# ethz-asl/infinitam

Hardware: AMD Instinct MI355X
Metric: fused depth frames/sec (640x480, hash TSDF) (higher is better)
Workload: dtype f32

## Files before the change

### include/itm_debug.h

```cpp
#ifndef ITM_DEBUG_H_
#define ITM_DEBUG_H_

#include "itm_hip.h"

#ifdef __cplusplus
extern "C" {
#endif

#define ITM_DEBUG_FORCE_GLOBAL_RANGE_ATOMICS 1
#define ITM_DEBUG_EXPLICIT_MARK_PREVIOUS 2
#define ITM_DEBUG_INTEGRATE_WORKGROUPS 3
#define ITM_DEBUG_NO_FUSED_PROJECTION 4
#define ITM_DEBUG_NO_DIRECTORY 5
#define ITM_DEBUG_NO_FUSED_RANGE_REDUCE 6
#define ITM_DEBUG_TWO_PASS_VISIBLE_LIST 7
#define ITM_DEBUG_SINGLE_PASS_RAYCAST 8
#define ITM_DEBUG_DENSE_GROUP_CULL 9
#define ITM_DEBUG_TRACKER_LAUNCH_PER_EVALUATION 10
#define ITM_DEBUG_TRACKER_HOST_COMMAND 11
#define ITM_DEBUG_SEPARATE_SWEEP 13
#define ITM_DEBUG_NO_SIDE_PROJECTION 14
#define ITM_DEBUG_DENSE_RANGE_REFILL 15
#define ITM_DEBUG_NO_SDF_MIRROR 12
#define ITM_DEBUG_DENSE_CLASSIFY 16
#define ITM_DEBUG_DENSE_NO_STRIPS 17
#define ITM_DEBUG_TRACKER_SESSION_UNUSABLE 18
#define ITM_DEBUG_NO_DEFERRED_FUSION 19
#define ITM_DEBUG_FORCE_LIST_STUCK 20
#define ITM_DEBUG_EXCHANGE_DEVICE_COPY 24
#define ITM_DEBUG_EXCHANGE_CORRUPT_WORD 25
#define ITM_DEBUG_MESH_ATTR_PER_VERTEX 26
#define ITM_DEBUG_MESH_INDEX_WEAK_HASH 27
int ITM_FN(debug_set)(int key, int value);
int ITM_FN(debug_checksum)(const int32_t* src, size_t words, int rounds, unsigned long long* dst, itm_stream stream);
int ITM_FN(debug_dense_classify_check)(int32_t out[4], int reset);
int ITM_FN(debug_column_cull_rows)(const float M_d[16], const float intr[4], int w, int h, float voxelSize, const int size[3],
                                   const int offset[3], int x0, int z, int* rlo, int* rhi);
int ITM_FN(debug_div32767)(const float* in, float* out, int n, itm_stream stream);
int ITM_FN(debug_divide)(int mode, const float* a, const float* b, const float* r, float* out, int n, itm_stream stream);


typedef int (*itm_icp_evaluate_fn)(void* user, int level, int iterationType, const float approxInvPose[16],
                                   float distThresh, itm_tracker_gh* out);
int ITM_FN(debug_icp_track)(const itm_tracker_config* cfg, const float M_d[16], itm_icp_evaluate_fn evaluate,
                            void* user, float M_d_out[16]);
int ITM_FN(debug_wicp_track)(const itm_tracker_config* cfg, const float M_d[16], itm_icp_evaluate_fn evaluate,
                             void* user, float M_d_out[16]);

#ifdef __cplusplus
}
#endif
#endif
```

### infinitam_amd/capi.py

```python
from __future__ import annotations

import ctypes as C
import os
import re
from dataclasses import dataclass, field
from typing import Optional

import numpy as np

VOXEL_S, VOXEL_F, VOXEL_S_RGB, VOXEL_F_RGB = 0, 1, 2, 3
INDEX_HASH, INDEX_DENSE = 0, 1
RENDER_SHADED_GREYSCALE, RENDER_COLOUR_FROM_VOLUME, RENDER_COLOUR_FROM_NORMAL = 0, 1, 2
(BUF_HASH_ENTRIES, BUF_EXCESS_LIST, BUF_VOXEL_BLOCKS, BUF_ALLOCATION_LIST, BUF_VISIBLE_IDS,
 BUF_VISIBLE_TYPE, BUF_RANGE_IMAGE, BUF_RAYCAST_RESULT, BUF_RAYCAST_IMAGE, BUF_FORWARD_PROJECTION,
 BUF_MISSING_POINTS, BUF_SWAP_STATES) = range(12)
ERR_INVALID, ERR_DEVICE, ERR_UNSUPPORTED = -1, -2, -3
MESH_NORMALS, MESH_COLOURS = 1, 2

VOXEL_NAMES = {VOXEL_S: "ITMVoxel_s", VOXEL_F: "ITMVoxel_f", VOXEL_S_RGB: "ITMVoxel_s_rgb",
               VOXEL_F_RGB: "ITMVoxel_f_rgb"}

HASH_ENTRY_DTYPE = np.dtype({"names": ["pos", "offset", "ptr"],
                             "formats": [("<i2", 3), "<i4", "<i4"],
                             "offsets": [0, 8, 12], "itemsize": 16})
# ... 211 lines not shown
    "host_free": (C.c_int, [_P]),
    "host_register": (C.c_int, [_P, C.c_size_t]),
    "host_unregister": (C.c_int, [_P]),
    "depth_stager_create": (C.c_int, [C.c_int, C.c_int, C.c_int, C.POINTER(_P)]),
    "depth_stager_destroy": (C.c_int, [_P]),
    "depth_stager_upload": (C.c_int, [_P, _P]),
    "depth_stager_acquire": (C.c_int, [_P, _P, C.POINTER(_P)]),
    "depth_stager_release": (C.c_int, [_P, _P]),
    "depth_stager_set_conversion": (C.c_int, [_P, C.c_int, C.c_float, C.c_float, C.c_float]),
    "depth_stager_acquire_depth": (C.c_int, [_P, _P, C.POINTER(_P), C.POINTER(_P)]),
    "depth_stager_pending": (C.c_int, [_P, C.POINTER(C.c_int), C.POINTER(C.c_int)]),
    "stream_create": (C.c_int, [C.POINTER(_P)]),
    "stream_destroy": (C.c_int, [_P]),
    "exchange_unique_id": (C.c_int, [C.POINTER(C.c_ubyte)]),
    "exchange_create": (C.c_int, [C.c_int, C.c_int, C.POINTER(C.c_ubyte), C.c_int, C.c_int, C.POINTER(_P)]),
    "exchange_destroy": (C.c_int, [_P]),
    "exchange_step": (C.c_int, [_P, _P, C.POINTER(C.c_float), _P]),
    "exchange_info": (C.c_int, [_P, C.POINTER(C.c_int), C.POINTER(C.c_int), C.POINTER(C.c_int), C.POINTER(C.c_int), C.POINTER(_P)]),
    "exchange_table": (C.c_int, [_P, _P, C.c_size_t]),
    "exchange_self_check": (C.c_int, [_P, C.POINTER(C.c_int), C.POINTER(C.c_int)]),
    "exchange_acquire": (C.c_int, [_P, _P, C.POINTER(_P), C.POINTER(C.c_longlong)]),
    "exchange_release": (C.c_int, [_P, _P]),
    "debug_checksum": (C.c_int, [_P, C.c_size_t, C.c_int, _P, _P]),
    "colour_tracker_create": (C.c_int, [C.POINTER(_P)]),
    "colour_tracker_destroy": (C.c_int, [_P]),
    "colour_tracker_prepare": (C.c_int, [_P, C.POINTER(ViewStruct), C.c_int, _P]),
    "colour_tracker_read_level": (C.c_int, [_P, C.c_int, _P, _P, _P, C.POINTER(C.c_int), C.POINTER(C.c_int), _P]),
    "colour_tracker_evaluate": (C.c_int, [_P, C.c_int, _P, _P, C.c_int, C.POINTER(C.c_float), C.c_int, C.c_int, C.POINTER(ColourEval), _P]),
    "colour_tracker_track_camera": (C.c_int, [_P, C.POINTER(TrackerConfig), C.POINTER(ViewStruct), _P, _P, _P, C.c_int,
                                              C.POINTER(C.c_float), _P]),
    "colour_tracker_evaluations": (C.c_int, [_P, C.POINTER(C.c_int)]),
    "ren_tracker_create": (C.c_int, [C.POINTER(_P)]),
    "ren_tracker_destroy": (C.c_int, [_P]),
    "ren_tracker_prepare": (C.c_int, [_P, C.POINTER(ViewStruct), _P, _P]),
    "ren_tracker_evaluate": (C.c_int, [_P, _P, C.POINTER(C.c_float), C.c_int, C.POINTER(RenEval), _P]),
    "ren_tracker_track_camera": (C.c_int, [_P, _P, C.POINTER(ViewStruct), C.POINTER(C.c_float), C.POINTER(C.c_int), _P]),
    "mesh_attributes": (C.c_int, [_P, _P, C.c_int, _P]),
    "mesh_download_attributes": (C.c_int, [_P, _P, _P, C.c_uint32, C.POINTER(C.c_uint32), _P]),
    "mesh_write_ply": (C.c_int, [_P, C.c_char_p, _P]),
    "mesh_index": (C.c_int, [_P, _P]),
    "mesh_index_info": (C.c_int, [_P, C.POINTER(C.c_uint32), C.POINTER(C.c_uint32), C.POINTER(_P), C.POINTER(_P), C.POINTER(_P), _P]),
    "mesh_download_indexed": (C.c_int, [_P, _P, _P, C.c_uint32, _P, C.c_uint32, C.POINTER(C.c_uint32), C.POINTER(C.c_uint32), _P]),
    "mesh_indexed_attributes": (C.c_int, [_P, _P, C.c_int, _P]),
    "mesh_download_indexed_attributes": (C.c_int, [_P, _P, _P, C.c_uint32, C.POINTER(C.c_uint32), _P]),
    "mesh_write_ply_indexed": (C.c_int, [_P, C.c_char_p, _P]),
    "mesh_write_obj_indexed": (C.c_int, [_P, C.c_char_p, _P]),
# ... 482 lines not shown
```

### infinitam_amd/csrc/itm_internal.h

```cpp
#pragma once

#include <hip/hip_runtime.h>

#include <string>
#include <vector>

#include "../../include/itm_hip.h"
#include "../../include/itm_debug.h"
#include "itm_types.h"

namespace itm {

struct SceneCounters {
  int32_t lastFreeBlockId;
  int32_t lastFreeExcessListId;
  int32_t noAllocRequests;
  int32_t statusFlags;
};
struct RenderCounters {
  int32_t noVisibleEntries;
  int32_t noFwdProjMissingPoints;
  int32_t noTotalPoints;
  int32_t noRenderingBlocks;
  int32_t rawVisibleCount;
// ... 65 lines not shown

struct itm_render_state {
  const itm_scene* scene = nullptr;
  int w = 0, h = 0;
  bool hash = false;
  int capIds = 0;
  bool listCoherent = true;
  bool lazyThisFrame = false;
  float2* range = nullptr;
  float4* raycast = nullptr;
  float4* fwdProj = nullptr;
  int32_t* missing = nullptr;
  uchar4* image = nullptr;
  int32_t* visibleIds = nullptr;
  uint8_t* visibleType = nullptr;
  itm::RenderCounters* counters = nullptr;
  uint4* projBuf = nullptr;
  uint2* rangePartials = nullptr;
  int32_t* pixScratch = nullptr;
  int32_t* pixChunk = nullptr;
  uint8_t* viewFlags = nullptr;
  int32_t* viewChunkVis = nullptr;
  bool denseRangeReady = false;
  hipStream_t sideStream = nullptr;
  hipEvent_t listReady = nullptr, projectionDone = nullptr;
  struct { bool valid = false; const float* depth = nullptr; int w = 0, h = 0; float M_d[16] = {}, intr_d[4] = {}; bool lazy = false; unsigned tableEpoch = 0; } ahead;
  struct { int stage = 0; itm_view view = {}; hipStream_t st = nullptr; } deferred;
};

namespace itm {

int set_error(int code, const std::string& msg);
int hip_fail(hipError_t e, const char* what, const char* file, int line);

#define ITM_HIP(call)                                                        \
  do {                                                                       \
    hipError_t _e = (call);                                                  \
    if (_e != hipSuccess) return itm::hip_fail(_e, #call, __FILE__, __LINE__); \
  } while (0)

#define ITM_LAUNCH_CHECK()                                                    \
  do {                                                                        \
    hipError_t _e = hipGetLastError();                                        \
    if (_e != hipSuccess) return itm::hip_fail(_e, "kernel launch", __FILE__, __LINE__); \
  } while (0)

// ... 26 lines not shown
int flush_deferred(itm_render_state* rs);
int enter_scene(const itm_scene* s, const itm_render_state* rs);
int flush_overlapping(const void* p, size_t bytes, hipStream_t st);
void forget_deferred(itm_render_state* rs);
extern int g_debug_no_deferred_fusion;
bool deferred_fusion_default();
extern int g_debug_force_list_stuck;
extern int g_debug_exchange_device_copy, g_debug_exchange_corrupt_word;
extern int g_debug_mesh_attr_per_vertex;
extern int g_debug_mesh_index_weak_hash;
int refuse_while_ahead(const itm_scene* s, const itm_render_state* rs, const char* what);

extern int g_debug_explicit_mark;
extern int g_debug_two_pass_visible_list;
extern int g_debug_integrate_wgs;
extern int g_debug_dense_group_cull;
extern int g_debug_dense_classify;
extern int g_debug_dense_no_strips;
extern int g_debug_tracker_launch_per_evaluation;
extern int g_debug_tracker_host_command;
extern int g_debug_tracker_session_unusable;
extern int g_debug_no_sdf_mirror;
extern int g_debug_separate_sweep;
int rebuild_sdf_mirror(itm_scene* s, hipStream_t st);
int launch_swap_after_allocation(itm_scene* s, itm_render_state* rs, hipStream_t st);
void free_swap_state(itm_scene* s);
int create_swap_state(itm_scene* s);
int live_hash_scenes(int device);
int accel_unfill(itm_scene* s, hipStream_t st);
int accel_place(itm_scene* s, const float* invM, hipStream_t st);
extern int g_debug_no_fused_projection;
int rebuild_head_bits(itm_scene* s, hipStream_t st);
extern int g_debug_no_directory;
int launch_request_stage(itm_scene* s, const itm_view* v, itm_render_state* rs, bool onlyVisible, bool fuseRangeInit, hipStream_t st);
int launch_sweep_stage(itm_scene* s, const itm_view* v, itm_render_state* rs, bool onlyVisible, hipStream_t st);
int launch_allocate(itm_scene* s, const itm_view* v, itm_render_state* rs, bool onlyVisible, bool fuseRangeInit, hipStream_t st);
int validate_allocate(const itm_scene* s, const itm_view* v, const itm_render_state* rs, bool onlyVisible);
int validate_integrate(const itm_scene* s, const itm_view* v);
int cancel_ahead(itm_scene* s, itm_render_state* rs, hipStream_t st);
int launch_integrate(itm_scene* s, const itm_view* v, itm_render_state* rs, hipStream_t st, bool fuseProjection = false);
bool can_fuse_projection(const itm_scene* s, const itm_render_state* rs);
int launch_find_visible(const itm_scene* s, const float* M, const float* intr, itm_render_state* rs, hipStream_t st);
int launch_expected_depths(const itm_scene* s, const float* M, const float* intr, itm_render_state* rs, bool rangeAlreadyInit, hipStream_t st, bool projected = false);
int launch_raycast(const itm_scene* s, const float* invM, const float* intr, itm_render_state* rs, float4* dst, hipStream_t st, bool reduceRange = false);
int launch_icp_maps(const itm_scene* s, const itm_view* v, itm_render_state* rs, float4* points, float4* normals, hipStream_t st, bool reduceRange = false,
                    itm_scene* sceneForNext = nullptr, const itm_view* next = nullptr);
// ... 6 lines not shown
```

### infinitam_amd/csrc/scene.hip

```cpp
#include <atomic>
#include <mutex>
#include <cstdio>
#include <cstring>
#include <new>

#include "itm_internal.h"

namespace itm {

static thread_local std::string g_last_error;

int set_error(int code, const std::string& msg) {
  g_last_error = msg;
  return code;
}
int hip_fail(hipError_t e, const char* what, const char* file, int line) {
  char buf[512];
  snprintf(buf, sizeof buf, "%s: %s (%s:%d)", what, hipGetErrorString(e), file, line);
  g_last_error = buf;
  return ITM_ERR_DEVICE;
}

hipEvent_t Profiler::get() {
  if (!pool.empty()) { hipEvent_t e = pool.back(); pool.pop_back(); return e; }
// ... 342 lines not shown
  (void)hipFree(s->hash); (void)hipFree(s->excessList); (void)hipFree(s->vba); (void)hipFree(s->allocList);
  (void)hipFree(s->counters); (void)hipFree(s->headBits); (void)hipFree(s->allocKey); (void)hipFree(s->chunkReq); (void)hipFree(s->chunkVis); (void)hipFree(s->chunkGran); (void)hipFree(s->chunkSweepDone); (void)hipFree(s->chunkKeptGran);
  (void)hipFree(s->dirPtr); (void)hipFree(s->dirSlot); (void)hipFree(s->sdfMirror); (void)hipFree(s->org.mTable); (void)hipFree(s->org.mPages); (void)hipFree(s->depthTiles);
  delete s;
}
static void free_rs(itm_render_state* r) {
  if (!r) return;
  bool haveScene;
  { std::lock_guard<std::mutex> lock(g_rsRegistryMutex); haveScene = r->scene != nullptr; }
  if (haveScene) (void)flush_deferred(r);
  {
    std::lock_guard<std::mutex> lock(g_rsRegistryMutex);
    itm_scene* s = const_cast<itm_scene*>(r->scene);
    if (s) {
      if (s->aheadRs == r) s->aheadRs = nullptr;
      for (size_t i = 0; i < s->renderStates.size(); ++i)
        if (s->renderStates[i] == r) { s->renderStates[i] = s->renderStates.back(); s->renderStates.pop_back(); break; }
    }
  }
  forget_deferred(r);
  (void)hipFree(r->range); (void)hipFree(r->raycast); (void)hipFree(r->fwdProj); (void)hipFree(r->missing);
  (void)hipFree(r->image); (void)hipFree(r->visibleIds); (void)hipFree(r->visibleType); (void)hipFree(r->counters);
  (void)hipFree(r->projBuf); (void)hipFree(r->rangePartials); (void)hipFree(r->pixScratch); (void)hipFree(r->pixChunk); (void)hipFree(r->viewFlags); (void)hipFree(r->viewChunkVis);
  if (r->sideStream) { (void)hipStreamSynchronize(r->sideStream); (void)hipStreamDestroy(r->sideStream); }
  if (r->listReady) (void)hipEventDestroy(r->listReady);
  if (r->projectionDone) (void)hipEventDestroy(r->projectionDone);
  delete r;
}

}

using namespace itm;

extern "C" {

const char* itm_version(void) { return "itm-hip 0.1 (gfx950)"; }
const char* itm_last_error(void) { return g_last_error.c_str(); }
int itm_uses_device_memory(void) { return 1; }
size_t itm_voxel_size_bytes(int t) {
  switch (t) {
    case ITM_VOXEL_S: return VoxelS::kBytes;
    case ITM_VOXEL_F: return VoxelF::kBytes;
    case ITM_VOXEL_S_RGB: return VoxelSRgb::kBytes;
    case ITM_VOXEL_F_RGB: return VoxelFRgb::kBytes;
  }
  return 0;
// ... 202 lines not shown

int itm_reset_scene(itm_scene* s, itm_stream stream) {
  if (!s) return set_error(ITM_ERR_INVALID, "null scene");
  hipStream_t st = as_stream(stream);
  if (s->deferredRs) { const int rc = flush_deferred(s->deferredRs); if (rc) return rc; }
  if (s->aheadRs) { const int rc = cancel_ahead(s, s->aheadRs, st); if (rc) return rc; }
  if (s->fatalHost && *s->fatalHost) { ITM_HIP(hipStreamSynchronize(st)); *s->fatalHost = 0; }
  const int grid = 2048;
  if (s->cfg.voxelType == ITM_VOXEL_S && (s->numVoxels % 4) == 0) {
    reset_voxels_s_x4_kernel<<<grid, 256, 0, st>>>((uint4*)s->vba, s->numVoxels / 4);
  } else {
    int rc = dispatch_voxel(s->cfg.voxelType, [&](auto vx) {
      using VX = decltype(vx);
      reset_voxels_kernel<VX><<<grid, 256, 0, st>>>(s->vba, s->numVoxels);
      return ITM_OK;
    });
    if (rc) return rc;
  }
  ITM_LAUNCH_CHECK();
  if (s->cfg.indexType == ITM_INDEX_HASH) {
    { int rc = accel_unfill(s, st); if (rc) return rc; }
    s->orgPlaced = false;
    ++s->tableEpoch;
    reset_hash_kernel<<<1024, 256, 0, st>>>(s->hash, s->noTotalEntries, s->excessList, s->cfg.excessNum, s->allocList,
                                            s->cfg.localBlockNum, s->allocKey, s->headBits, (s->cfg.bucketNum + 31) / 32, s->chunkReq, s->numChunks * 4, s->counters);
  } else {
    reset_dense_kernel<<<1, 1, 0, st>>>(s->allocList, s->counters);
  }
  ITM_LAUNCH_CHECK();
  return ITM_OK;
}

int itm_render_state_create(const itm_scene* s, int w, int h, itm_render_state** out) {
  if (!s || !out || w <= 0 || h <= 0) return set_error(ITM_ERR_INVALID, "bad argument");
  if ((long long)w * h >= (1ll << 24)) return set_error(ITM_ERR_INVALID, "image too large");
  itm_render_state* r = new (std::nothrow) itm_render_state();
  if (!r) return set_error(ITM_ERR_DEVICE, "out of host memory");
  r->scene = s; r->w = w; r->h = h;
  r->hash = s->cfg.indexType == ITM_INDEX_HASH;
  r->capIds = r->hash ? s->cfg.localBlockNum : 0;
  size_t P = (size_t)w * h;
  hipError_t e = hipSuccess;
  auto alloc = [&](void** p, size_t bytes) { if (e == hipSuccess) e = hipMalloc(p, bytes ? bytes : 16); };
  alloc((void**)&r->range, P * 8);
  alloc((void**)&r->raycast, P * 16);
  alloc((void**)&r->fwdProj, P * 16);
  alloc((void**)&r->missing, P * 4);
  alloc((void**)&r->image, P * 4);
  alloc((void**)&r->counters, sizeof(RenderCounters));
  alloc((void**)&r->pixScratch, P * 4);
  alloc((void**)&r->pixChunk, ((P + kSweepChunk - 1) / kSweepChunk) * 4 + 16);
  if (r->hash) {
    alloc((void**)&r->visibleIds, (size_t)r->capIds * 4);
    alloc((void**)&r->visibleType, (size_t)s->noTotalEntries);
    alloc((void**)&r->projBuf, (size_t)r->capIds * 32);
    if ((size_t)((w + 7) / 8) * ((h + 7) / 8) * 8 <= 150 * 1024) alloc((void**)&r->rangePartials, (size_t)64 * ((w + 7) / 8) * ((h + 7) / 8) * 8);
  }
  if (e != hipSuccess) { free_rs(r); return hip_fail(e, "hipMalloc(render state)", __FILE__, __LINE__); }
  e = hipMemset(r->counters, 0, sizeof(RenderCounters));
  if (e == hipSuccess) e = hipMemset(r->raycast, 0, P * 16);
  if (e == hipSuccess) e = hipMemset(r->fwdProj, 0, P * 16);
  if (e == hipSuccess) e = hipMemset(r->missing, 0, P * 4);
  if (e == hipSuccess) e = hipMemset(r->image, 0, P * 4);
  if (e == hipSuccess && r->hash) e = hipMemset(r->visibleIds, 0, (size_t)r->capIds * 4);
  if (e == hipSuccess && r->hash) e = hipMemset(r->visibleType, 0, (size_t)s->noTotalEntries);
  if (e != hipSuccess) { free_rs(r); return hip_fail(e, "hipMemset(render state)", __FILE__, __LINE__); }
  fill_range_kernel<<<256, 256, 0, 0>>>(r->range, (int)P, s->prm.viewFrustum_min, s->prm.viewFrustum_max);
  e = hipDeviceSynchronize();
  if (e != hipSuccess) { free_rs(r); return hip_fail(e, "init range image", __FILE__, __LINE__); }
  { std::lock_guard<std::mutex> lock(g_rsRegistryMutex); s->renderStates.push_back(r); }
  *out = r;
  return ITM_OK;
}
int itm_render_state_destroy(itm_render_state* r) { free_rs(r); return ITM_OK; }

int itm_debug_div32767(const float* in, float* out, int n, itm_stream st) {
  if (!in || !out || n < 0) return set_error(ITM_ERR_INVALID, "bad argument");
  div32767_kernel<<<(n + 255) / 256, 256, 0, as_stream(st)>>>(in, out, n);
  ITM_LAUNCH_CHECK();
  return ITM_OK;
}

int itm_debug_divide(int mode, const float* a, const float* b, const float* r, float* out, int n, itm_stream st) {
  if (!a || !b || !out || n < 0 || mode < 1 || mode > 4 || (mode == 4 && !r)) return set_error(ITM_ERR_INVALID, "bad argument");
  divide_kernel<<<(n + 255) / 256, 256, 0, as_stream(st)>>>(mode, a, b, r, out, n);
  ITM_LAUNCH_CHECK();
  return ITM_OK;
}
// ... 154 lines not shown
```

### infinitam_amd/csrc/visualise.hip

```cpp
#include <cstdlib>
#include <cstring>

#include "itm_internal.h"
#include "alloc_device.h"
#include "shading_device.h"
#include "range_device.h"
#include "wave_utils.h"


namespace itm {

#ifndef ITM_MIRROR_FLOAT_TYPES
#define ITM_MIRROR_FLOAT_TYPES 0
#endif

int g_debug_force_global_range = 0;
int g_debug_no_directory = 0;
int g_debug_no_sdf_mirror = 0;
int g_debug_no_fused_range_reduce = 0;
int g_debug_single_pass_raycast = 0;
int g_debug_no_side_projection = 0;
int g_debug_dense_range_refill = 0;

__global__ void __launch_bounds__(256) range_init_kernel(float2* __restrict__ img, int n, float a, float b, RenderCounters* rc) {
  const int stride = gridDim.x * blockDim.x;
  for (int i = blockIdx.x * blockDim.x + threadIdx.x; i < n; i += stride) img[i] = make_float2(a, b);
  if (blockIdx.x == 0 && threadIdx.x == 0) { rc->noRenderingBlocks = 0; rc->renderingBlocksAccepted = -1; }
}

__device__ inline void merge_box(float2* __restrict__ range, int W, const Projected& r) {
  const uint32_t z0 = __float_as_uint(r.z0), z1 = __float_as_uint(r.z1);
  for (int y = r.uly; y <= r.lry; ++y)
    for (int x = r.ulx; x <= r.lrx; ++x) {
      uint32_t* px = (uint32_t*)&range[x + y * W];
      atomicMin(px, z0);
      atomicMax(px + 1, z1);
    }
}

__global__ void __launch_bounds__(256) project_fill_kernel(const int32_t* __restrict__ ids, RenderCounters* __restrict__ rc,
                                                           const uint4* __restrict__ hash, float2* __restrict__ range,
                                                           uint4* __restrict__ projBuf, ProjParams p) {
  const int nv = rc->noVisibleEntries;
// ... 206 lines not shown
  __syncthreads();
  if (tid < 4) {
    const int cx = tx * 2 + (tid & 1), cy = ty * 2 + (tid >> 1);
    const float2 r = make_float2(__uint_as_float(capCells[2 * tid]), __uint_as_float(capCells[2 * tid + 1]));
    cellRange[tid] = r;
    if (cx < f.RW && cy < f.RH) f.range[cx + cy * W] = r;
  }
}

constexpr float kSilhouetteSpread = 0.3f;
constexpr int kSilhouettePrio = 3;
#ifndef ITM_EXP_RAYCAST_STAMPS
#define ITM_EXP_RAYCAST_STAMPS 0
#endif
#if ITM_EXP_RAYCAST_STAMPS
__device__ unsigned long long g_rayStamps[8192 * 4];
#define ITM_RS(...) __VA_ARGS__
#else
#define ITM_RS(...)
#endif

struct AheadRequest { RequestArgs ra; AllocParams ap; int rayTiles, reqTilesX; };

template <class VX, bool DENSE, bool REDUCE, bool PARK, bool AHEAD = false, int MIRROR = 0>
__global__ void __launch_bounds__(256) raycast_kernel(VolumeView volIn, const float2* __restrict__ range, float4* __restrict__ out, RayParams p, RangeFuse fuse, AheadRequest ahead) {
  if constexpr (AHEAD) {
    if ((int)blockIdx.x >= ahead.rayTiles) {
      const int r = (int)blockIdx.x - ahead.rayTiles;
      request_tile<false, false, true>(r % ahead.reqTilesX, r / ahead.reqTilesX, ahead.ra, ahead.ap);
      return;
    }
  }
  VolumeViewM<MIRROR> vol(volIn);
  if constexpr (MIRROR == 0) vol.sdfMirror = nullptr;
  const int lane = threadIdx.x & 63, wave = threadIdx.x >> 6;
  const int tilesX = (p.W + 15) / 16;
  const int tx = blockIdx.x % tilesX, ty = blockIdx.x / tilesX;
  const int lx = lane & 15, ly = wave * 4 + (lane >> 4);
  const int x = tx * 16 + lx;
  const int y = ty * 16 + ly;
  const bool inside = x < p.W && y < p.H;
  __shared__ float2 cellRange[4];
  __shared__ float4 parkState[PARK ? 256 : 1];
  __shared__ int parkSource[PARK ? 256 : 1];
  __shared__ int parkCount;
  if (PARK && threadIdx.x == 0) parkCount = 0;
  ITM_RS(unsigned long long* stamp = g_rayStamps + (size_t)((blockIdx.x * 4 + wave) & 8191) * 4; if (lane == 0) stamp[0] = __builtin_amdgcn_s_memrealtime();)
  float2 mm = make_float2(0.0f, 0.0f);
  if constexpr (REDUCE) {
    reduce_own_cells(fuse, tx, ty, p.W, cellRange);
    __syncthreads();
    if (inside) mm = cellRange[(lx >> 3) + 2 * (ly >> 3)];
  } else {
    if (PARK) __syncthreads();
    if (inside) mm = range[(x >> 3) + (y >> 3) * p.W];
  }
  ITM_RS(if (lane == 0) stamp[1] = __builtin_amdgcn_s_memrealtime();)
  if (!DENSE && __any(inside && mm.y - mm.x > kSilhouetteSpread)) __builtin_amdgcn_s_setprio(kSilhouettePrio);
  bool parked = false;
  if (inside) {
// ... 1 lines not shown
    if (!parked) out[x + y * p.W] = r;
    else if constexpr (PARK) {
      const int slot = atomicAdd(&parkCount, 1);
      parkState[slot] = r;
      parkSource[slot] = ly * 16 + lx;
    }
  }
  ITM_RS(if (lane == 0) { stamp[2] = __builtin_amdgcn_s_memrealtime(); stamp[3] = 0; })
  if constexpr (PARK) {
    __syncthreads();
    const int n = parkCount;
    if ((int)threadIdx.x < n) {
      const float4 q = parkState[threadIdx.x];
      const int src = parkSource[threadIdx.x];
      const int qx = tx * 16 + (src & 15), qy = ty * 16 + (src >> 4);
      float2 m2;
      if constexpr (REDUCE) m2 = cellRange[((src & 15) >> 3) + 2 * (src >> 7)];
      else m2 = range[(qx >> 3) + (qy >> 3) * p.W];
      const RayResume rr{q.x, q.y, q.z, q.w};
      bool again;
      out[qx + qy * p.W] = march_ray<VX, DENSE, kParkedLookahead, false>(qx, qy, vol, p, m2, &rr, again);
    }
    ITM_RS(if (lane == 0) stamp[3] = __builtin_amdgcn_s_memrealtime() | ((unsigned long long)(wave == 0 ? n : 0) << 52);)
  }
}
#if ITM_EXP_RAYCAST_STAMPS
extern "C" int itm_debug_read_raycast_stamps(unsigned long long* dst, int n) { return (int)hipMemcpyFromSymbol(dst, HIP_SYMBOL(g_rayStamps), (size_t)n * 8); }
#endif

int launch_raycast(const itm_scene* s, const float* invM, const float* intr, itm_render_state* rs, float4* dst, hipStream_t st, bool reduceRange, const AheadRequest* aheadIn) {
  RayParams p; make_ray_params(s, invM, intr, rs->w, rs->h, p);
  const VolumeView vol = make_volume(s);
  const int rayTiles = ((rs->w + 15) / 16) * ((rs->h + 15) / 16);
  const bool dense = s->cfg.indexType == ITM_INDEX_DENSE;
  RangeFuse fuse{rs->rangePartials, rs->counters, rs->projBuf, rs->range, (rs->w + 7) / 8, (rs->h + 7) / 8, s->cfg.maxRenderingBlocks};
  const bool park = !dense && vol.dirPtr != nullptr && !g_debug_single_pass_raycast;
  AheadRequest ahead;
  memset(&ahead, 0, sizeof ahead);
  int reqTiles = 0;
  if (aheadIn && !dense) { ahead = *aheadIn; ahead.rayTiles = rayTiles; reqTiles = ahead.reqTilesX * ((ahead.ap.H + 15) / 16); }
  const dim3 grid(rayTiles + reqTiles);
  KernelTimer tk(s, ITM_TK_RAYCAST, st);
  const int mirrorForm = (!vol.sdfMirror || !park) ? 0 : (vol.org.mMaxPages < 0 ? 1 : 2);
  int rc = dispatch_voxel(s->cfg.voxelType, [&](auto vx) {
    using VX = decltype(vx);
    constexpr bool kMayMirror = VX::kShort || ITM_MIRROR_FLOAT_TYPES;
#define ITM_RC(RED, PRK, AHD, MIR) raycast_kernel<VX, false, RED, PRK, AHD, MIR><<<grid, 256, 0, st>>>(vol, rs->range, dst, p, fuse, ahead)
#define ITM_RC_MIRROR(RED, AHD) do { if (kMayMirror && mirrorForm == 1) ITM_RC(RED, true, AHD, (kMayMirror ? 1 : 0)); else if (kMayMirror && mirrorForm == 2) ITM_RC(RED, true, AHD, (kMayMirror ? 2 : 0)); else ITM_RC(RED, true, AHD, 0); } while (0)
    if (dense) raycast_kernel<VX, true, false, false><<<grid, 256, 0, st>>>(vol, rs->range, dst, p, fuse, ahead);
    else if (reqTiles) {
      if (park) { if (reduceRange) ITM_RC_MIRROR(true, true); else ITM_RC_MIRROR(false, true); }
      else if (reduceRange) ITM_RC(true, false, true, 0);
      else ITM_RC(false, false, true, 0);
    }
    else if (park) { if (reduceRange) ITM_RC_MIRROR(true, false); else ITM_RC_MIRROR(false, false); }
    else if (reduceRange) ITM_RC(true, false, false, 0);
    else ITM_RC(false, false, false, 0);
#undef ITM_RC_MIRROR
#undef ITM_RC
    return ITM_OK;
  });
  if (rc) return rc;
  ITM_LAUNCH_CHECK();
  return ITM_OK;
}
int launch_raycast(const itm_scene* s, const float* invM, const float* intr, itm_render_state* rs, float4* dst, hipStream_t st, bool reduceRange) {
  return launch_raycast(s, invM, intr, rs, dst, st, reduceRange, nullptr);
}

__device__ inline void nt_store(float4* p, float4 v) { __builtin_nontemporal_store(v.x, &p->x); __builtin_nontemporal_store(v.y, &p->y); __builtin_nontemporal_store(v.z, &p->z); __builtin_nontemporal_store(v.w, &p->w); }
__device__ inline void nt_store(uchar4* p, uchar4 v) { __builtin_nontemporal_store(*(unsigned int*)&v, (unsigned int*)p); }

__global__ void __launch_bounds__(256) icp_maps_kernel(const float4* __restrict__ rays, float4* __restrict__ points,
                                                       float4* __restrict__ normals, uchar4* __restrict__ image, RayParams p) {
  __shared__ float4 hits[20][20];
  const int lane = threadIdx.x & 63, wave = threadIdx.x >> 6;
  const int lx = lane & 15, ly = wave * 4 + (lane >> 4);
  const int x = blockIdx.x * 16 + lx, y = blockIdx.y * 16 + ly;
  const bool inside = x < p.W && y < p.H;
  if (inside) hits[2 + ly][2 + lx] = rays[x + y * p.W];
  if (threadIdx.x < 128) {
    const int strip = threadIdx.x >> 5, k = threadIdx.x & 31;
    int hx, hy;
    if (strip < 2) { hx = strip == 0 ? (k & 1) : 18 + (k & 1); hy = 2 + (k >> 1); }
    else { hy = strip == 2 ? (k & 1) : 18 + (k & 1); hx = 2 + (k >> 1); }
    const int gx = (int)blockIdx.x * 16 + hx - 2, gy = (int)blockIdx.y * 16 + hy - 2;
    if (gx >= 0 && gx < p.W && gy >= 0 && gy < p.H) hits[hy][hx] = rays[gx + gy * p.W];
  }
  __syncthreads();
  if (!inside) return;
  const int loc = x + y * p.W;
  const float4 r = hits[2 + ly][2 + lx];
  bool found = r.w > 0.0f;
  float nx = 0, ny = 0, nz = 0, angle = 0;
  const int ox = (int)blockIdx.x * 16 - 2, oy = (int)blockIdx.y * 16 - 2;
  if (found) found = normal_from_hits_at([&](int qx, int qy) { return hits[qy - oy][qx - ox]; }, x, y, p.W, p.H, p.voxelSize, p.lx, p.ly, p.lz, nx, ny, nz, angle);
  if (found) {
    nt_store(&image[loc], grey_pixel(angle));
    nt_store(&points[loc], make_float4(r.x * p.voxelSize, r.y * p.voxelSize, r.z * p.voxelSize, 1.0f));
    nt_store(&normals[loc], make_float4(nx, ny, nz, 0.0f));
  } else {
    const float4 inv = make_float4(0.0f, 0.0f, 0.0f, -1.0f);
    nt_store(&points[loc], inv); nt_store(&normals[loc], inv); nt_store(&image[loc], make_uchar4(0, 0, 0, 0));
  }
}

__global__ void __launch_bounds__(256) icp_maps_init_next_kernel(const float4* __restrict__ rays, float4* __restrict__ points, float4* __restrict__ normals,
                                                                 uchar4* __restrict__ image, RayParams p, float2* __restrict__ range, RenderCounters* __restrict__ rcnt) {
  const int lane = threadIdx.x & 63, wave = threadIdx.x >> 6;
  if (blockIdx.x == 0 && blockIdx.y == 0 && threadIdx.x == 0) { rcnt->noRenderingBlocks = 0; rcnt->renderingBlocksAccepted = -1; }
  const int x = blockIdx.x * 16 + (lane & 15);
  const int y = blockIdx.y * 16 + wave * 4 + (lane >> 4);
  if (x >= p.W || y >= p.H) return;
  const int loc = x + y * p.W;
  range[loc] = make_float2(999999.9f, 0.05f);
  const float4 r = rays[loc];
  bool found = r.w > 0.0f;
  float nx = 0, ny = 0, nz = 0, angle = 0;
  if (found) found = normal_from_hits(rays, x, y, p.W, p.H, p.voxelSize, p.lx, p.ly, p.lz, nx, ny, nz, angle);
  if (found) {
    nt_store(&image[loc], grey_pixel(angle));
    nt_store(&points[loc], make_float4(r.x * p.voxelSize, r.y * p.voxelSize, r.z * p.voxelSize, 1.0f));
    nt_store(&normals[loc], make_float4(nx, ny, nz, 0.0f));
  } else {
    const float4 inv = make_float4(0.0f, 0.0f, 0.0f, -1.0f);
    nt_store(&points[loc], inv); nt_store(&normals[loc], inv); nt_store(&image[loc], make_uchar4(0, 0, 0, 0));
  }
}

int prepare_request_stage(itm_scene* s, const itm_view* v, itm_render_state* rs, hipStream_t st, AllocParams& p, RequestArgs& ra, bool& lazy);

int launch_icp_maps(const itm_scene* s, const itm_view* v, itm_render_state* rs, float4* points, float4* normals, hipStream_t st, bool reduceRange,
                    itm_scene* sceneForNext, const itm_view* next) {
  float invM[16];
  if (!invert4(v->M_d, invM)) return set_error(ITM_ERR_INVALID, "pose matrix is singular");
  AheadRequest ahead;
  bool issueAhead = false;
  if (next && sceneForNext) {
    bool lazy = false;
    int rc = prepare_request_stage(sceneForNext, next, rs, st, ahead.ap, ahead.ra, lazy);
    if (rc) return rc;
    issueAhead = lazy;
    ahead.reqTilesX = (next->w + 15) / 16;
  }
  int rc = launch_raycast(s, invM, v->intr_d, rs, rs->raycast, st, reduceRange, issueAhead ? &ahead : nullptr);
  if (rc) return rc;
  RayParams p; make_ray_params(s, invM, v->intr_d, rs->w, rs->h, p);
  const dim3 grid((rs->w + 15) / 16, (rs->h + 15) / 16);
  KernelTimer tk(s, ITM_TK_ICP_MAPS, st);
  if (issueAhead) {
    icp_maps_init_next_kernel<<<grid, 256, 0, st>>>(rs->raycast, points, normals, rs->image, p, rs->range, rs->counters);
    rs->ahead.tableEpoch = sceneForNext->tableEpoch;
    sceneForNext->aheadRs = rs;
    rs->ahead.valid = true; rs->ahead.depth = next->depth; rs->ahead.w = next->w; rs->ahead.h = next->h; rs->ahead.lazy = true;
    memcpy(rs->ahead.M_d, next->M_d, 64); memcpy(rs->ahead.intr_d, next->intr_d, 16);
  } else {
    icp_maps_kernel<<<grid, 256, 0, st>>>(rs->raycast, points, normals, rs->image, p);
  }
  ITM_LAUNCH_CHECK();
  return ITM_OK;
}

template <class VX, bool DENSE>
__global__ void __launch_bounds__(256) render_image_kernel(VolumeView vol, const float4* __restrict__ rays, uchar4* __restrict__ out, int type, RayParams p) {
  const int lane = threadIdx.x & 63, wave = threadIdx.x >> 6;
  const int x = blockIdx.x * 16 + (lane & 15);
  const int y = blockIdx.y * 16 + wave * 4 + (lane >> 4);
  if (x >= p.W || y >= p.H) return;
  const int loc = x + y * p.W;
  const float4 r = rays[loc];
  bool found = r.w > 0;
  float nx = 0, ny = 0, nz = 0, angle = 0;
  if (found) found = normal_from_sdf<VX, DENSE>(vol, r.x, r.y, r.z, p, nx, ny, nz, angle);
  if (!found) { out[loc] = make_uchar4(0, 0, 0, 0); return; }
  if (type == ITM_RENDER_COLOUR_FROM_VOLUME) {
    const float4 c = colour_at<VX, DENSE>(vol, r.x, r.y, r.z);
    out[loc] = make_uchar4((unsigned char)(c.x * 255.0f), (unsigned char)(c.y * 255.0f), (unsigned char)(c.z * 255.0f), 255);
  } else if (type == ITM_RENDER_COLOUR_FROM_NORMAL) {
    unsigned char* o = (unsigned char*)&out[loc];
    o[0] = (unsigned char)((0.3f + (-nx + 1.0f) * 0.35f) * 255.0f);
    o[1] = (unsigned char)((0.3f + (-ny + 1.0f) * 0.35f) * 255.0f);
    o[2] = (unsigned char)((0.3f + (-nz + 1.0f) * 0.35f) * 255.0f);
// ... 36 lines not shown
  if (key == ITM_DEBUG_EXPLICIT_MARK_PREVIOUS) { g_debug_explicit_mark = value; return ITM_OK; }
  if (key == ITM_DEBUG_INTEGRATE_WORKGROUPS) { g_debug_integrate_wgs = value; return ITM_OK; }
  if (key == ITM_DEBUG_NO_FUSED_PROJECTION) { g_debug_no_fused_projection = value; return ITM_OK; }
  if (key == ITM_DEBUG_NO_DIRECTORY) { g_debug_no_directory = value; return ITM_OK; }
  if (key == ITM_DEBUG_NO_FUSED_RANGE_REDUCE) { g_debug_no_fused_range_reduce = value; return ITM_OK; }
  if (key == ITM_DEBUG_TWO_PASS_VISIBLE_LIST) { g_debug_two_pass_visible_list = value; return ITM_OK; }
  if (key == ITM_DEBUG_SINGLE_PASS_RAYCAST) { g_debug_single_pass_raycast = value; return ITM_OK; }
  if (key == ITM_DEBUG_DENSE_GROUP_CULL) { g_debug_dense_group_cull = value; return ITM_OK; }
  if (key == ITM_DEBUG_TRACKER_LAUNCH_PER_EVALUATION) { g_debug_tracker_launch_per_evaluation = value; return ITM_OK; }
  if (key == ITM_DEBUG_TRACKER_HOST_COMMAND) { g_debug_tracker_host_command = value; return ITM_OK; }
  if (key == ITM_DEBUG_NO_SDF_MIRROR) { g_debug_no_sdf_mirror = value; return ITM_OK; }
  if (key == ITM_DEBUG_SEPARATE_SWEEP) { g_debug_separate_sweep = value; return ITM_OK; }
  if (key == ITM_DEBUG_NO_SIDE_PROJECTION) { g_debug_no_side_projection = value; return ITM_OK; }
  if (key == ITM_DEBUG_DENSE_RANGE_REFILL) { g_debug_dense_range_refill = value; return ITM_OK; }
  if (key == ITM_DEBUG_DENSE_CLASSIFY) { g_debug_dense_classify = value; return ITM_OK; }
  if (key == ITM_DEBUG_TRACKER_SESSION_UNUSABLE) { g_debug_tracker_session_unusable = value; return ITM_OK; }
  if (key == ITM_DEBUG_DENSE_NO_STRIPS) { g_debug_dense_no_strips = value; return ITM_OK; }
  if (key == ITM_DEBUG_NO_DEFERRED_FUSION) { g_debug_no_deferred_fusion = value; return ITM_OK; }
  if (key == ITM_DEBUG_FORCE_LIST_STUCK) { g_debug_force_list_stuck = value; return ITM_OK; }
  if (key == ITM_DEBUG_EXCHANGE_DEVICE_COPY) { g_debug_exchange_device_copy = value; return ITM_OK; }
  if (key == ITM_DEBUG_EXCHANGE_CORRUPT_WORD) { g_debug_exchange_corrupt_word = value; return ITM_OK; }
  if (key == ITM_DEBUG_MESH_ATTR_PER_VERTEX) { g_debug_mesh_attr_per_vertex = value; return ITM_OK; }
  if (key == ITM_DEBUG_MESH_INDEX_WEAK_HASH) { g_debug_mesh_index_weak_hash = value; return ITM_OK; }
  return set_error(ITM_ERR_INVALID, "unknown debug key");
}

int itm_find_surface(const itm_scene* s, const float M[16], const float intr[4], itm_render_state* rs, itm_stream stream) {
  if (!s || !M || !intr || !rs) return set_error(ITM_ERR_INVALID, "null argument");
  if (rs->scene != s) return set_error(ITM_ERR_INVALID, "render state belongs to another scene");
  { const int rc = enter_scene(s, rs); if (rc) return rc; }
  float invM[16];
  if (!invert4(M, invM)) return set_error(ITM_ERR_INVALID, "pose matrix is singular");
  return launch_raycast(s, invM, intr, rs, rs->raycast, as_stream(stream));
}

int itm_render_image(const itm_scene* s, const float M[16], const float intr[4], itm_render_state* rs, uint8_t* out, int type, itm_stream stream) {
  if (!s || !M || !intr || !rs) return set_error(ITM_ERR_INVALID, "null argument");
  if (rs->scene != s) return set_error(ITM_ERR_INVALID, "render state belongs to another scene");
  { const int rc = enter_scene(s, rs); if (rc) return rc; }
  return launch_render_image(s, M, intr, rs, out ? (uchar4*)out : rs->image, type, as_stream(stream));
}

int itm_process_frame(itm_scene* s, const itm_view* v, itm_render_state* rs, float* points, float* normals, itm_stream stream) {
  return itm_process_frame_ahead(s, v, nullptr, rs, points, normals, stream);
}

int itm_process_frame_ahead(itm_scene* s, const itm_view* v, const itm_view* next, itm_render_state* rs, float* points, float* normals, itm_stream stream) {
// ... 31 lines not shown
```

Baseline: 12680.

## Reorder raycast tiles so previously slow tiles dispatch first

The parked raycast kernel records per tile whether any rays needed the slow parked path. The last block of the ICP-maps kernel then builds a permutation that puts those flagged tiles first, and the next frame's raycast reads its tile index from that permutation. The aim is to start long-running tiles early and shorten the tail of unbalanced workgroups. The cost is an extra indirection per block, a serial per-thread scan in one block, and a dependence on frame-to-frame coherence. The order is invalidated when the hash table is reset.

```diff
diff --git a/include/itm_debug.h b/include/itm_debug.h
--- a/include/itm_debug.h
+++ b/include/itm_debug.h
@@ -31,7 +31,9 @@
 #define ITM_DEBUG_EXCHANGE_CORRUPT_WORD 25
 #define ITM_DEBUG_MESH_ATTR_PER_VERTEX 26
 #define ITM_DEBUG_MESH_INDEX_WEAK_HASH 27
+#define ITM_DEBUG_IDENTITY_TILE_ORDER 28
 int ITM_FN(debug_set)(int key, int value);
+int ITM_FN(debug_tile_order)(const itm_render_state* rs, int32_t info[4], uint16_t* order, uint8_t* slow, int cap);
 int ITM_FN(debug_checksum)(const int32_t* src, size_t words, int rounds, unsigned long long* dst, itm_stream stream);
 int ITM_FN(debug_dense_classify_check)(int32_t out[4], int reset);
 int ITM_FN(debug_column_cull_rows)(const float M_d[16], const float intr[4], int w, int h, float voxelSize, const int size[3],
diff --git a/infinitam_amd/capi.py b/infinitam_amd/capi.py
--- a/infinitam_amd/capi.py
+++ b/infinitam_amd/capi.py
@@ -257,6 +257,7 @@
     "exchange_acquire": (C.c_int, [_P, _P, C.POINTER(_P), C.POINTER(C.c_longlong)]),
     "exchange_release": (C.c_int, [_P, _P]),
     "debug_checksum": (C.c_int, [_P, C.c_size_t, C.c_int, _P, _P]),
+    "debug_tile_order": (C.c_int, [_P, C.POINTER(C.c_int32), _P, _P, C.c_int]),
     "colour_tracker_create": (C.c_int, [C.POINTER(_P)]),
     "colour_tracker_destroy": (C.c_int, [_P]),
     "colour_tracker_prepare": (C.c_int, [_P, C.POINTER(ViewStruct), C.c_int, _P]),
diff --git a/infinitam_amd/csrc/itm_internal.h b/infinitam_amd/csrc/itm_internal.h
--- a/infinitam_amd/csrc/itm_internal.h
+++ b/infinitam_amd/csrc/itm_internal.h
@@ -111,6 +111,11 @@
   uint8_t* viewFlags = nullptr;
   int32_t* viewChunkVis = nullptr;
   bool denseRangeReady = false;
+  uint8_t* tileSlow = nullptr;
+  uint16_t* tileOrder = nullptr;
+  int rayTiles = 0;
+  struct { int w = 0, h = 0, buf = -1; } tileOrderValid;
+  long long orderedCasts = 0;
   hipStream_t sideStream = nullptr;
   hipEvent_t listReady = nullptr, projectionDone = nullptr;
   struct { bool valid = false; const float* depth = nullptr; int w = 0, h = 0; float M_d[16] = {}, intr_d[4] = {}; bool lazy = false; unsigned tableEpoch = 0; } ahead;
@@ -183,6 +188,7 @@
 extern int g_debug_tracker_session_unusable;
 extern int g_debug_no_sdf_mirror;
 extern int g_debug_separate_sweep;
+extern int g_debug_identity_tile_order;
 int rebuild_sdf_mirror(itm_scene* s, hipStream_t st);
 int launch_swap_after_allocation(itm_scene* s, itm_render_state* rs, hipStream_t st);
 void free_swap_state(itm_scene* s);
diff --git a/infinitam_amd/csrc/scene.hip b/infinitam_amd/csrc/scene.hip
--- a/infinitam_amd/csrc/scene.hip
+++ b/infinitam_amd/csrc/scene.hip
@@ -388,6 +388,7 @@
   (void)hipFree(r->range); (void)hipFree(r->raycast); (void)hipFree(r->fwdProj); (void)hipFree(r->missing);
   (void)hipFree(r->image); (void)hipFree(r->visibleIds); (void)hipFree(r->visibleType); (void)hipFree(r->counters);
   (void)hipFree(r->projBuf); (void)hipFree(r->rangePartials); (void)hipFree(r->pixScratch); (void)hipFree(r->pixChunk); (void)hipFree(r->viewFlags); (void)hipFree(r->viewChunkVis);
+  (void)hipFree(r->tileSlow); (void)hipFree(r->tileOrder);
   if (r->sideStream) { (void)hipStreamSynchronize(r->sideStream); (void)hipStreamDestroy(r->sideStream); }
   if (r->listReady) (void)hipEventDestroy(r->listReady);
   if (r->projectionDone) (void)hipEventDestroy(r->projectionDone);
@@ -636,6 +637,7 @@
     { int rc = accel_unfill(s, st); if (rc) return rc; }
     s->orgPlaced = false;
     ++s->tableEpoch;
+    { std::lock_guard<std::mutex> lock(g_rsRegistryMutex); for (itm_render_state* r : s->renderStates) r->tileOrderValid.buf = -1; }
     reset_hash_kernel<<<1024, 256, 0, st>>>(s->hash, s->noTotalEntries, s->excessList, s->cfg.excessNum, s->allocList,
                                             s->cfg.localBlockNum, s->allocKey, s->headBits, (s->cfg.bucketNum + 31) / 32, s->chunkReq, s->numChunks * 4, s->counters);
   } else {
@@ -670,6 +672,12 @@
     alloc((void**)&r->projBuf, (size_t)r->capIds * 32);
     if ((size_t)((w + 7) / 8) * ((h + 7) / 8) * 8 <= 150 * 1024) alloc((void**)&r->rangePartials, (size_t)64 * ((w + 7) / 8) * ((h + 7) / 8) * 8);
   }
+  const size_t rayTiles = (size_t)((w + 15) / 16) * ((h + 15) / 16), rayTilesPadded = (rayTiles + 1) & ~(size_t)1;
+  if (r->hash && rayTiles <= 65535) {
+    r->rayTiles = (int)rayTiles;
+    alloc((void**)&r->tileSlow, rayTiles);
+    alloc((void**)&r->tileOrder, 2 * rayTilesPadded * sizeof(uint16_t));
+  }
   if (e != hipSuccess) { free_rs(r); return hip_fail(e, "hipMalloc(render state)", __FILE__, __LINE__); }
   e = hipMemset(r->counters, 0, sizeof(RenderCounters));
   if (e == hipSuccess) e = hipMemset(r->raycast, 0, P * 16);
@@ -678,6 +686,8 @@
   if (e == hipSuccess) e = hipMemset(r->image, 0, P * 4);
   if (e == hipSuccess && r->hash) e = hipMemset(r->visibleIds, 0, (size_t)r->capIds * 4);
   if (e == hipSuccess && r->hash) e = hipMemset(r->visibleType, 0, (size_t)s->noTotalEntries);
+  if (e == hipSuccess && r->rayTiles) e = hipMemset(r->tileSlow, 0, rayTiles);
+  if (e == hipSuccess && r->rayTiles) e = hipMemset(r->tileOrder, 0, 2 * rayTilesPadded * sizeof(uint16_t));
   if (e != hipSuccess) { free_rs(r); return hip_fail(e, "hipMemset(render state)", __FILE__, __LINE__); }
   fill_range_kernel<<<256, 256, 0, 0>>>(r->range, (int)P, s->prm.viewFrustum_min, s->prm.viewFrustum_max);
   e = hipDeviceSynchronize();
diff --git a/infinitam_amd/csrc/visualise.hip b/infinitam_amd/csrc/visualise.hip
--- a/infinitam_amd/csrc/visualise.hip
+++ b/infinitam_amd/csrc/visualise.hip
@@ -19,6 +19,7 @@
 int g_debug_no_sdf_mirror = 0;
 int g_debug_no_fused_range_reduce = 0;
 int g_debug_single_pass_raycast = 0;
+int g_debug_identity_tile_order = 0;
 int g_debug_no_side_projection = 0;
 int g_debug_dense_range_refill = 0;
 
@@ -271,8 +272,10 @@
 
 struct AheadRequest { RequestArgs ra; AllocParams ap; int rayTiles, reqTilesX; };
 
-template <class VX, bool DENSE, bool REDUCE, bool PARK, bool AHEAD = false, int MIRROR = 0>
-__global__ void __launch_bounds__(256) raycast_kernel(VolumeView volIn, const float2* __restrict__ range, float4* __restrict__ out, RayParams p, RangeFuse fuse, AheadRequest ahead) {
+struct TileOrder { const uint32_t* order; uint8_t* slow; };
+
+template <class VX, bool DENSE, bool REDUCE, bool PARK, bool AHEAD = false, int MIRROR = 0, bool ORDERED = false>
+__global__ void __launch_bounds__(256) raycast_kernel(VolumeView volIn, const float2* __restrict__ range, float4* __restrict__ out, RayParams p, RangeFuse fuse, AheadRequest ahead, TileOrder ord) {
   if constexpr (AHEAD) {
     if ((int)blockIdx.x >= ahead.rayTiles) {
       const int r = (int)blockIdx.x - ahead.rayTiles;
@@ -284,7 +287,16 @@
   if constexpr (MIRROR == 0) vol.sdfMirror = nullptr;
   const int lane = threadIdx.x & 63, wave = threadIdx.x >> 6;
   const int tilesX = (p.W + 15) / 16;
-  const int tx = blockIdx.x % tilesX, ty = blockIdx.x / tilesX;
+  unsigned tile = blockIdx.x;
+  if constexpr (ORDERED) {
+    if (ord.order) {
+      const uint32_t two = ord.order[blockIdx.x >> 1];
+      const unsigned last = (unsigned)(tilesX * ((p.H + 15) / 16) - 1);
+      tile = (blockIdx.x & 1) ? two >> 16 : two & 0xffffu;
+      tile = tile < last ? tile : last;
+    }
+  }
+  const int tx = tile % tilesX, ty = tile / tilesX;
   const int lx = lane & 15, ly = wave * 4 + (lane >> 4);
   const int x = tx * 16 + lx;
   const int y = ty * 16 + ly;
@@ -332,13 +344,15 @@
       out[qx + qy * p.W] = march_ray<VX, DENSE, kParkedLookahead, false>(qx, qy, vol, p, m2, &rr, again);
     }
     ITM_RS(if (lane == 0) stamp[3] = __builtin_amdgcn_s_memrealtime() | ((unsigned long long)(wave == 0 ? n : 0) << 52);)
+    if constexpr (ORDERED) { if (threadIdx.x == 0) ord.slow[tile] = n > 0 ? 1 : 0; }
   }
 }
 #if ITM_EXP_RAYCAST_STAMPS
 extern "C" int itm_debug_read_raycast_stamps(unsigned long long* dst, int n) { return (int)hipMemcpyFromSymbol(dst, HIP_SYMBOL(g_rayStamps), (size_t)n * 8); }
 #endif
 
-int launch_raycast(const itm_scene* s, const float* invM, const float* intr, itm_render_state* rs, float4* dst, hipStream_t st, bool reduceRange, const AheadRequest* aheadIn) {
+int launch_raycast(const itm_scene* s, const float* invM, const float* intr, itm_render_state* rs, float4* dst, hipStream_t st, bool reduceRange, const AheadRequest* aheadIn,
+                   bool* keepTileOrder = nullptr) {
   RayParams p; make_ray_params(s, invM, intr, rs->w, rs->h, p);
   const VolumeView vol = make_volume(s);
   const int rayTiles = ((rs->w + 15) / 16) * ((rs->h + 15) / 16);
@@ -352,12 +366,22 @@
   const dim3 grid(rayTiles + reqTiles);
   KernelTimer tk(s, ITM_TK_RAYCAST, st);
   const int mirrorForm = (!vol.sdfMirror || !park) ? 0 : (vol.org.mMaxPages < 0 ? 1 : 2);
+  const bool ordered = keepTileOrder && park && rs->rayTiles == rayTiles && !g_debug_identity_tile_order;
+  TileOrder ord{nullptr, rs->tileSlow};
+  if (ordered && rs->tileOrderValid.buf >= 0 && rs->tileOrderValid.w == rs->w && rs->tileOrderValid.h == rs->h) {
+    ord.order = (const uint32_t*)(rs->tileOrder + (size_t)rs->tileOrderValid.buf * ((rayTiles + 1) & ~1));
+    ++rs->orderedCasts;
+  }
+  if (!ordered) rs->tileOrderValid.buf = -1;
+  if (keepTileOrder) *keepTileOrder = ordered;
   int rc = dispatch_voxel(s->cfg.voxelType, [&](auto vx) {
     using VX = decltype(vx);
     constexpr bool kMayMirror = VX::kShort || ITM_MIRROR_FLOAT_TYPES;
-#define ITM_RC(RED, PRK, AHD, MIR) raycast_kernel<VX, false, RED, PRK, AHD, MIR><<<grid, 256, 0, st>>>(vol, rs->range, dst, p, fuse, ahead)
-#define ITM_RC_MIRROR(RED, AHD) do { if (kMayMirror && mirrorForm == 1) ITM_RC(RED, true, AHD, (kMayMirror ? 1 : 0)); else if (kMayMirror && mirrorForm == 2) ITM_RC(RED, true, AHD, (kMayMirror ? 2 : 0)); else ITM_RC(RED, true, AHD, 0); } while (0)
-    if (dense) raycast_kernel<VX, true, false, false><<<grid, 256, 0, st>>>(vol, rs->range, dst, p, fuse, ahead);
+#define ITM_RC_O(RED, PRK, AHD, MIR, ORD) raycast_kernel<VX, false, RED, PRK, AHD, MIR, ORD><<<grid, 256, 0, st>>>(vol, rs->range, dst, p, fuse, ahead, ord)
+#define ITM_RC(RED, PRK, AHD, MIR) ITM_RC_O(RED, PRK, AHD, MIR, false)
+#define ITM_RC_PARK(RED, AHD, MIR) do { if (ordered) ITM_RC_O(RED, true, AHD, MIR, true); else ITM_RC_O(RED, true, AHD, MIR, false); } while (0)
+#define ITM_RC_MIRROR(RED, AHD) do { if (kMayMirror && mirrorForm == 1) ITM_RC_PARK(RED, AHD, (kMayMirror ? 1 : 0)); else if (kMayMirror && mirrorForm == 2) ITM_RC_PARK(RED, AHD, (kMayMirror ? 2 : 0)); else ITM_RC_PARK(RED, AHD, 0); } while (0)
+    if (dense) raycast_kernel<VX, true, false, false><<<grid, 256, 0, st>>>(vol, rs->range, dst, p, fuse, ahead, ord);
     else if (reqTiles) {
       if (park) { if (reduceRange) ITM_RC_MIRROR(true, true); else ITM_RC_MIRROR(false, true); }
       else if (reduceRange) ITM_RC(true, false, true, 0);
@@ -367,7 +391,9 @@
     else if (reduceRange) ITM_RC(true, false, false, 0);
     else ITM_RC(false, false, false, 0);
 #undef ITM_RC_MIRROR
+#undef ITM_RC_PARK
 #undef ITM_RC
+#undef ITM_RC_O
     return ITM_OK;
   });
   if (rc) return rc;
@@ -381,8 +407,31 @@
 __device__ inline void nt_store(float4* p, float4 v) { __builtin_nontemporal_store(v.x, &p->x); __builtin_nontemporal_store(v.y, &p->y); __builtin_nontemporal_store(v.z, &p->z); __builtin_nontemporal_store(v.w, &p->w); }
 __device__ inline void nt_store(uchar4* p, uchar4 v) { __builtin_nontemporal_store(*(unsigned int*)&v, (unsigned int*)p); }
 
+__device__ inline void build_tile_order(const uint8_t* __restrict__ slow, uint16_t* __restrict__ order, int n) {
+  __shared__ int waveFlagged[4];
+  const int lane = threadIdx.x & 63, wave = threadIdx.x >> 6;
+  const int per = (n + 255) / 256;
+  const int lo = min((int)threadIdx.x * per, n), hi = min(lo + per, n);
+  int mine = 0;
+  for (int i = lo; i < hi; ++i) mine += slow[i] != 0;
+  int incl = mine;
+#pragma unroll
+  for (int o = 1; o < 64; o <<= 1) { const int v = __shfl_up(incl, o, 64); if (lane >= o) incl += v; }
+  if (lane == 63) waveFlagged[wave] = incl;
+  __syncthreads();
+  int before = incl - mine, flagged = 0;
+#pragma unroll
+  for (int w = 0; w < 4; ++w) { const int c = waveFlagged[w]; if (w < wave) before += c; flagged += c; }
+  for (int i = lo; i < hi; ++i) {
+    const bool f = slow[i] != 0;
+    order[f ? before : flagged + (i - before)] = (uint16_t)i;
+    before += f;
+  }
+}
+struct TileOrderBuild { const uint8_t* slow; uint16_t* order; int n; };
+
 __global__ void __launch_bounds__(256) icp_maps_kernel(const float4* __restrict__ rays, float4* __restrict__ points,
-                                                       float4* __restrict__ normals, uchar4* __restrict__ image, RayParams p) {
+                                                       float4* __restrict__ normals, uchar4* __restrict__ image, RayParams p, TileOrderBuild tiles) {
   __shared__ float4 hits[20][20];
   const int lane = threadIdx.x & 63, wave = threadIdx.x >> 6;
   const int lx = lane & 15, ly = wave * 4 + (lane >> 4);
@@ -398,44 +447,49 @@
     if (gx >= 0 && gx < p.W && gy >= 0 && gy < p.H) hits[hy][hx] = rays[gx + gy * p.W];
   }
   __syncthreads();
-  if (!inside) return;
-  const int loc = x + y * p.W;
-  const float4 r = hits[2 + ly][2 + lx];
-  bool found = r.w > 0.0f;
-  float nx = 0, ny = 0, nz = 0, angle = 0;
-  const int ox = (int)blockIdx.x * 16 - 2, oy = (int)blockIdx.y * 16 - 2;
-  if (found) found = normal_from_hits_at([&](int qx, int qy) { return hits[qy - oy][qx - ox]; }, x, y, p.W, p.H, p.voxelSize, p.lx, p.ly, p.lz, nx, ny, nz, angle);
-  if (found) {
-    nt_store(&image[loc], grey_pixel(angle));
-    nt_store(&points[loc], make_float4(r.x * p.voxelSize, r.y * p.voxelSize, r.z * p.voxelSize, 1.0f));
-    nt_store(&normals[loc], make_float4(nx, ny, nz, 0.0f));
-  } else {
-    const float4 inv = make_float4(0.0f, 0.0f, 0.0f, -1.0f);
-    nt_store(&points[loc], inv); nt_store(&normals[loc], inv); nt_store(&image[loc], make_uchar4(0, 0, 0, 0));
-  }
+  if (inside) {
+    const int loc = x + y * p.W;
+    const float4 r = hits[2 + ly][2 + lx];
+    bool found = r.w > 0.0f;
+    float nx = 0, ny = 0, nz = 0, angle = 0;
+    const int ox = (int)blockIdx.x * 16 - 2, oy = (int)blockIdx.y * 16 - 2;
+    if (found) found = normal_from_hits_at([&](int qx, int qy) { return hits[qy - oy][qx - ox]; }, x, y, p.W, p.H, p.voxelSize, p.lx, p.ly, p.lz, nx, ny, nz, angle);
+    if (found) {
+      nt_store(&image[loc], grey_pixel(angle));
+      nt_store(&points[loc], make_float4(r.x * p.voxelSize, r.y * p.voxelSize, r.z * p.voxelSize, 1.0f));
+      nt_store(&normals[loc], make_float4(nx, ny, nz, 0.0f));
+    } else {
+      const float4 inv = make_float4(0.0f, 0.0f, 0.0f, -1.0f);
+      nt_store(&points[loc], inv); nt_store(&normals[loc], inv); nt_store(&image[loc], make_uchar4(0, 0, 0, 0));
+    }
+  }
+  if (tiles.slow && blockIdx.x == gridDim.x - 1 && blockIdx.y == gridDim.y - 1) build_tile_order(tiles.slow, tiles.order, tiles.n);
 }
 
 __global__ void __launch_bounds__(256) icp_maps_init_next_kernel(const float4* __restrict__ rays, float4* __restrict__ points, float4* __restrict__ normals,
-                                                                 uchar4* __restrict__ image, RayParams p, float2* __restrict__ range, RenderCounters* __restrict__ rcnt) {
+                                                                 uchar4* __restrict__ image, RayParams p, float2* __restrict__ range, RenderCounters* __restrict__ rcnt,
+                                                                 TileOrderBuild tiles) {
   const int lane = threadIdx.x & 63, wave = threadIdx.x >> 6;
   if (blockIdx.x == 0 && blockIdx.y == 0 && threadIdx.x == 0) { rcnt->noRenderingBlocks = 0; rcnt->renderingBlocksAccepted = -1; }
   const int x = blockIdx.x * 16 + (lane & 15);
   const int y = blockIdx.y * 16 + wave * 4 + (lane >> 4);
-  if (x >= p.W || y >= p.H) return;
-  const int loc = x + y * p.W;
-  range[loc] = make_float2(999999.9f, 0.05f);
-  const float4 r = rays[loc];
-  bool found = r.w > 0.0f;
-  float nx = 0, ny = 0, nz = 0, angle = 0;
-  if (found) found = normal_from_hits(rays, x, y, p.W, p.H, p.voxelSize, p.lx, p.ly, p.lz, nx, ny, nz, angle);
-  if (found) {
-    nt_store(&image[loc], grey_pixel(angle));
-    nt_store(&points[loc], make_float4(r.x * p.voxelSize, r.y * p.voxelSize, r.z * p.voxelSize, 1.0f));
-    nt_store(&normals[loc], make_float4(nx, ny, nz, 0.0f));
-  } else {
-    const float4 inv = make_float4(0.0f, 0.0f, 0.0f, -1.0f);
-    nt_store(&points[loc], inv); nt_store(&normals[loc], inv); nt_store(&image[loc], make_uchar4(0, 0, 0, 0));
-  }
+  if (x < p.W && y < p.H) {
+    const int loc = x + y * p.W;
+    range[loc] = make_float2(999999.9f, 0.05f);
+    const float4 r = rays[loc];
+    bool found = r.w > 0.0f;
+    float nx = 0, ny = 0, nz = 0, angle = 0;
+    if (found) found = normal_from_hits(rays, x, y, p.W, p.H, p.voxelSize, p.lx, p.ly, p.lz, nx, ny, nz, angle);
+    if (found) {
+      nt_store(&image[loc], grey_pixel(angle));
+      nt_store(&points[loc], make_float4(r.x * p.voxelSize, r.y * p.voxelSize, r.z * p.voxelSize, 1.0f));
+      nt_store(&normals[loc], make_float4(nx, ny, nz, 0.0f));
+    } else {
+      const float4 inv = make_float4(0.0f, 0.0f, 0.0f, -1.0f);
+      nt_store(&points[loc], inv); nt_store(&normals[loc], inv); nt_store(&image[loc], make_uchar4(0, 0, 0, 0));
+    }
+  }
+  if (tiles.slow && blockIdx.x == gridDim.x - 1 && blockIdx.y == gridDim.y - 1) build_tile_order(tiles.slow, tiles.order, tiles.n);
 }
 
 int prepare_request_stage(itm_scene* s, const itm_view* v, itm_render_state* rs, hipStream_t st, AllocParams& p, RequestArgs& ra, bool& lazy);
@@ -453,21 +507,26 @@
     issueAhead = lazy;
     ahead.reqTilesX = (next->w + 15) / 16;
   }
-  int rc = launch_raycast(s, invM, v->intr_d, rs, rs->raycast, st, reduceRange, issueAhead ? &ahead : nullptr);
+  bool keepTileOrder = false;
+  int rc = launch_raycast(s, invM, v->intr_d, rs, rs->raycast, st, reduceRange, issueAhead ? &ahead : nullptr, &keepTileOrder);
   if (rc) return rc;
+  const int nextBuf = rs->tileOrderValid.buf == 0 ? 1 : 0;
+  TileOrderBuild tiles{nullptr, nullptr, 0};
+  if (keepTileOrder) tiles = TileOrderBuild{rs->tileSlow, rs->tileOrder + (size_t)nextBuf * ((rs->rayTiles + 1) & ~1), rs->rayTiles};
   RayParams p; make_ray_params(s, invM, v->intr_d, rs->w, rs->h, p);
   const dim3 grid((rs->w + 15) / 16, (rs->h + 15) / 16);
   KernelTimer tk(s, ITM_TK_ICP_MAPS, st);
   if (issueAhead) {
-    icp_maps_init_next_kernel<<<grid, 256, 0, st>>>(rs->raycast, points, normals, rs->image, p, rs->range, rs->counters);
+    icp_maps_init_next_kernel<<<grid, 256, 0, st>>>(rs->raycast, points, normals, rs->image, p, rs->range, rs->counters, tiles);
     rs->ahead.tableEpoch = sceneForNext->tableEpoch;
     sceneForNext->aheadRs = rs;
     rs->ahead.valid = true; rs->ahead.depth = next->depth; rs->ahead.w = next->w; rs->ahead.h = next->h; rs->ahead.lazy = true;
     memcpy(rs->ahead.M_d, next->M_d, 64); memcpy(rs->ahead.intr_d, next->intr_d, 16);
   } else {
-    icp_maps_kernel<<<grid, 256, 0, st>>>(rs->raycast, points, normals, rs->image, p);
+    icp_maps_kernel<<<grid, 256, 0, st>>>(rs->raycast, points, normals, rs->image, p, tiles);
   }
   ITM_LAUNCH_CHECK();
+  if (keepTileOrder) { rs->tileOrderValid.w = rs->w; rs->tileOrderValid.h = rs->h; rs->tileOrderValid.buf = nextBuf; }
   return ITM_OK;
 }
 
@@ -550,7 +609,22 @@
   if (key == ITM_DEBUG_EXCHANGE_CORRUPT_WORD) { g_debug_exchange_corrupt_word = value; return ITM_OK; }
   if (key == ITM_DEBUG_MESH_ATTR_PER_VERTEX) { g_debug_mesh_attr_per_vertex = value; return ITM_OK; }
   if (key == ITM_DEBUG_MESH_INDEX_WEAK_HASH) { g_debug_mesh_index_weak_hash = value; return ITM_OK; }
+  if (key == ITM_DEBUG_IDENTITY_TILE_ORDER) { g_debug_identity_tile_order = value; return ITM_OK; }
   return set_error(ITM_ERR_INVALID, "unknown debug key");
+}
+
+int itm_debug_tile_order(const itm_render_state* rs, int32_t info[4], uint16_t* order, uint8_t* slow, int cap) {
+  if (!rs || !info) return set_error(ITM_ERR_INVALID, "null argument");
+  if (rs->scene) { const int rc = enter_scene(rs->scene, rs); if (rc) return rc; }
+  ITM_HIP(hipDeviceSynchronize());
+  const bool valid = rs->rayTiles > 0 && rs->tileOrderValid.buf >= 0 && rs->tileOrderValid.w == rs->w && rs->tileOrderValid.h == rs->h;
+  info[0] = rs->rayTiles; info[1] = valid ? 1 : 0; info[2] = valid ? rs->tileOrderValid.buf : -1;
+  info[3] = (int32_t)(rs->orderedCasts < 0x7fffffff ? rs->orderedCasts : 0x7fffffff);
+  if (valid && cap >= rs->rayTiles) {
+    if (order) ITM_HIP(hipMemcpy(order, rs->tileOrder + (size_t)rs->tileOrderValid.buf * ((rs->rayTiles + 1) & ~1), (size_t)rs->rayTiles * sizeof(uint16_t), hipMemcpyDeviceToHost));
+    if (slow) ITM_HIP(hipMemcpy(slow, rs->tileSlow, (size_t)rs->rayTiles, hipMemcpyDeviceToHost));
+  }
+  return ITM_OK;
 }
 
 int itm_find_surface(const itm_scene* s, const float M[16], const float intr[4], itm_render_state* rs, itm_stream stream) {
```

New measurement: 12540. 0.989x the previous value.
